# ActiveVisionLab/gaussctrl

Measured on AMD Instinct MI355X. Metric: edited views/sec @512x512 (ControlNet denoise + splat render+bwd), higher is better.
Workload: dtype bf16

## Files before the change

gaussctrl_amd/csrc/dn_gemm.hip:

```cpp
#include "dn_gemm_kernels.h"

namespace {

struct GemmVariant {
    int force_mt;
    int use8;
    int convsplit;
    bool no_wg2, no_persist, full_epilogue, no_lean_ln, tap_outer;
    int forced_pw, slice_mt, epi_abl;
    int undefined;
};
GemmVariant decode_variant(int kv)
{
    const auto bit = [kv](int b) { return (kv & b) != 0; };
    const auto field = [kv](int mask, int shift) { return (kv & mask) >> shift; };
    constexpr int flags = GC_GEMM_VAR_K4_ONLY | GC_GEMM_VAR_FORCE_K8 | GC_GEMM_VAR_NO_CONV_SLICES | GC_GEMM_VAR_NO_SMALL_CONV_SLICES | GC_GEMM_VAR_NO_WG2 |
                          GC_GEMM_VAR_NO_PERSIST | GC_GEMM_VAR_FULL_EPILOGUE | GC_GEMM_VAR_NO_LEAN_LN | GC_GEMM_VAR_TAP_OUTER;
    return {field(GC_GEMM_VAR_MT_MASK, GC_GEMM_VAR_MT_SHIFT), bit(GC_GEMM_VAR_K4_ONLY) ? 0 : bit(GC_GEMM_VAR_FORCE_K8) ? 2 : 1,
            bit(GC_GEMM_VAR_NO_CONV_SLICES) ? 0 : bit(GC_GEMM_VAR_NO_SMALL_CONV_SLICES) ? 1 : 2,
            bit(GC_GEMM_VAR_NO_WG2), bit(GC_GEMM_VAR_NO_PERSIST), bit(GC_GEMM_VAR_FULL_EPILOGUE), bit(GC_GEMM_VAR_NO_LEAN_LN), bit(GC_GEMM_VAR_TAP_OUTER),
            field(GC_GEMM_VAR_PW_MASK, GC_GEMM_VAR_PW_SHIFT), field(GC_GEMM_VAR_SLICE_MT_MASK, GC_GEMM_VAR_SLICE_MT_SHIFT), field(GC_GEMM_VAR_EPI_ABL_MASK, GC_GEMM_VAR_EPI_ABL_SHIFT),
            kv & ~(flags | GC_GEMM_VAR_MT_MASK | GC_GEMM_VAR_PW_MASK | GC_GEMM_VAR_SLICE_MT_MASK | GC_GEMM_VAR_EPI_ABL_MASK)};
}

int choose_splits(int64_t blocks, int nk)
{
    if (blocks >= 128 || nk < 32) return 1;
    int s = (int)((448 + blocks - 1) / blocks);
    if (s > nk / 8) s = nk / 8;
    if (s > 16) s = 16;
    return s < 2 ? 1 : s;
}

int choose_mt(int64_t M, int64_t N, int ntw, bool forced)
{
// ... 200 lines not shown
}

extern "C" int gc_dn_gemm_chan_parts_layout(const gc_gemm_desc *d, int64_t *rows_per_slab, int *nslab, int *col_tile)
{
    GC_REQUIRE(d && rows_per_slab && nslab && col_tile, "null argument");
    *rows_per_slab = 0; *nslab = 0; *col_tile = 0;
    if (d->M <= 0 || d->N <= 0 || d->K <= 0 || d->rows_per_batch <= 0) return GC_OK;
    const GemmVariant v = decode_variant(d->kernel_variant);
    Sel sel;
    select(d, v, &sel, true);
    chan_parts_layout(d, v, sel, rows_per_slab, nslab, col_tile);
    return GC_OK;
}

namespace {
struct Route { Sel sel; int lnk, persist; };
void route(const gc_gemm_desc *d, const GemmVariant &v, Route *r)
{
    Sel &sel = r->sel;
    select(d, v, &sel, d->out_chan_parts != nullptr);
    if (d->out_chan_parts && sel.mt8 == 1) sel.mt8 = 2;
    const bool fuse = d->ln_row_stats || d->out_row_stats || d->out_group_stats;
    r->lnk = (sel.mt8 && sel.splits == 1) ? ln_lean_kind(d, v) : 0;
    r->persist = 0;
    if (sel.mt8 == 4 && sel.ntw == 4 && sel.mode == 0 && sel.splits == 1 && d->K % 64 == 0 && d->K <= 64 * 24 && (!fuse || r->lnk == 2) && !d->out_chan_parts &&
        !d->rowvec && !d->out_t && !d->out_f32 && d->out && d->act != 2 && !v.no_persist) {
        const int64_t tiles = ((d->M + 255) / 256) * ((d->N + 32 * sel.ntw - 1) / (32 * sel.ntw));
        if (tiles > 256) r->persist = 256;
    }
}
}

extern "C" int gc_dn_gemm_selection(const gc_gemm_desc *d, gc_gemm_selection *out)
{
    GC_REQUIRE(d && out, "null argument");
    GC_REQUIRE(d->M > 0 && d->N > 0 && d->K > 0, "empty problem");
    const GemmVariant v = decode_variant(d->kernel_variant);
    if (const int rc = refuse_variant_bits(__func__, v.undefined)) return rc;
    *out = gc_gemm_selection{};
    int64_t rows = 0; int ns = 0, ct = 0;
    if (d->fp8) {
        GC_REQUIRE(d->K % 128 == 0, "fp8: K % 128 == 0");
        SelQ q;
        select_fp8(d, v, &q, false);
        out->kernel = GC_GEMM_SEL_FP8; out->m_tiles = q.mt; out->splits = q.splits; out->ntw = q.ntw;
        if (d->out_chan_parts) {
            chan_parts_layout(d, v, Sel{}, &rows, &ns, &ct);
            out->parts = rows > 0 ? (q.splits > 1 ? 1 : 2) : -1;
        }
        return GC_OK;
    }
    Route r;
    route(d, v, &r);
    out->kernel = !r.sel.mt8 ? GC_GEMM_SEL_K4 : r.sel.splits > 1 ? GC_GEMM_SEL_K8_SLICED : GC_GEMM_SEL_K8;
    out->m_tiles = r.sel.mt8; out->splits = r.sel.splits; out->ntw = r.sel.ntw; out->ln_kind = r.lnk; out->persist = r.persist;
    if (d->out_chan_parts) {
        chan_parts_layout(d, v, r.sel, &rows, &ns, &ct);
        out->parts = rows > 0 ? (r.sel.splits > 1 ? 1 : 2) : -1;
    }
    return GC_OK;
}

extern "C" int gc_dn_gemm(const gc_gemm_desc *d, void *stream)
{
    GC_REQUIRE(d && d->W && d->A, "null descriptor / operand");
    GC_REQUIRE(d->M > 0 && d->N > 0 && d->K > 0, "empty problem");
    GC_REQUIRE(d->K % 8 == 0, "K must be a multiple of 8 (pad channels on the host)");
    GC_REQUIRE(d->N % 4 == 0, "N must be a multiple of 4 (pad output channels on the host)");
    GC_REQUIRE(d->dtype == DT_BF16 || d->dtype == DT_F16, "dtype must be 0 (bf16) or 1 (f16)");
    const GemmVariant v = decode_variant(d->kernel_variant);
// ... 66 lines not shown
        const int ntw = q.ntw, mt = q.mt;
        g.splits = q.splits; g.tiles_per_split = q.tps; g.ws = q.splits > 1 ? (float *)d->workspace : nullptr;
        GC_REQUIRE(!d->out_chan_parts || q.splits > 1 || (d->mode == 1 && !fuse_of(g)), "fp8: channel partials come from k-sliced problems and fast convs");
        const int64_t nbn_q = (d->N + 32 * ntw - 1) / (32 * ntw), nbm_q = (d->M + 64 * mt - 1) / (64 * mt);
        const dim3 gq((unsigned)(nbm_q * nbn_q), (unsigned)q.splits);
        g.pw = pw_of(d, v, nbm_q, nbn_q, nbm_q * nbn_q * q.splits, 32, 64 * mt, 32 * ntw);
        dn_gemm_launch_fp8(g, d->dtype, d->mode == 1 ? 2 : 3, ntw, mt, gq, s);
        if (q.splits > 1) { if (g.chan_parts) dn_gemm_launch_splitk_epilogue_cs(g, d->dtype, s); else dn_gemm_launch_splitk_epilogue(g, d->dtype, s); }
        return gc::check_launch("gc_dn_gemm(fp8)");
    }
    g.splits = sel.splits; g.tiles_per_split = sel.tps; g.ws = (float *)d->workspace;
    const int bn = 32 * sel.ntw;
    const int64_t nbn = (d->N + bn - 1) / bn;
    g.persist = rt.persist;
    const int lnk = rt.lnk;
    if (d->w_set_rows > 0 || d->softmax_keys > 0) {
        GC_REQUIRE(lnk != 0, "weight sets / softmax_keys need a lean LayerNorm-fold problem (K % 64 == 0 linear with ln_row_stats or out_row_stats, no forced variant)");
        GC_REQUIRE(d->w_set_rows == 0 || (d->w_set_rows % (64 * sel.mt8) == 0 && d->M % d->w_set_rows == 0), "w_set_rows must be a multiple of the row tile and divide M");
    }
    if (sel.mt8) {
        const int64_t nbm8 = (d->M + 64 * sel.mt8 - 1) / (64 * sel.mt8);
        const dim3 grid8((unsigned)(nbm8 * nbn), (unsigned)sel.splits);
        g.pw = pw_of(d, v, nbm8, nbn, g.persist ? 8 * 32 : nbm8 * nbn * sel.splits, sel.mt8 == 1 ? 64 : 32, 64 * sel.mt8, bn);
        if (lnk) dn_gemm_launch_ln(g, d->dtype, lnk, lean_of(g, sel.mode) && g.persist == 0, sel.ntw, sel.mt8, grid8, s);
        else if (fuse_of(g)) dn_gemm_launch_fuse(g, d->dtype, sel.mode, sel.ntw, sel.mt8 < 2 ? 2 : sel.mt8, grid8, s);
        else if (g.chan_parts && sel.splits == 1) dn_gemm_launch_cs(g, d->dtype, sel.mode, sel.ntw, sel.mt8, grid8, s);
        else if (lean_of(g, sel.mode) && g.persist == 0 && !v.full_epilogue) dn_gemm_launch_lean(g, d->dtype, sel.mode, sel.ntw, sel.mt8, grid8, s);
        else dn_gemm_launch_plain(g, d->dtype, sel.mode, sel.ntw, sel.mt8, grid8, s);
    } else {
        const int64_t nbm = (d->M + BM - 1) / BM;
        const dim3 grid((unsigned)(nbm * nbn), (unsigned)sel.splits);
        g.pw = pw_of(d, v, nbm, nbn, nbm * nbn * sel.splits, 64, BM, bn);
        if (fuse_of(g)) dn_gemm_launch_fuse(g, d->dtype, sel.mode, sel.ntw, 0, grid, s); else dn_gemm_launch_plain(g, d->dtype, sel.mode, sel.ntw, 0, grid, s);
    }
    if (sel.splits > 1) { if (g.chan_parts) dn_gemm_launch_splitk_epilogue_cs(g, d->dtype, s); else dn_gemm_launch_splitk_epilogue(g, d->dtype, s); }
    return gc::check_launch("gc_dn_gemm");
}
```

gaussctrl_amd/csrc/dn_gemm_kernels.h:

```cpp
#pragma once
#include "dn_common.h"
#include <type_traits>

namespace dng {
struct GemmArgs {
    int64_t M, N, K;
    const void *A; int64_t lda;
    int B, Hi, Wi, Cin, Ho, Wo, stride, ups, pad;
    const void *W;
    const float *bias;
    const float *rowvec; int64_t ld_rowvec; int64_t rows_per_batch;
    const void *residual; int64_t ldr;
    float out_scale;
    int act, geglu;
    void *out; int64_t ldc; int out_f32;
    void *out_t; int64_t ldt; int64_t t_batch_stride; int64_t t_col0;
    int splits; int tiles_per_split;
    int persist;
    float *ws;
    const void *zeros;
    const float *row_stats; int row_stat_slots; const float *colsum; float ln_eps, ln_inv_k;
    float *out_row_stats;
    float *out_group_stats;
    int gn_groups, gn_cpg;
// ... 640 lines not shown
__device__ __forceinline__ void glds16_s(const void *sbase, unsigned voff, unsigned lds_dst)
{
    asm volatile("s_mov_b32 m0, %2\n\ts_nop 0\n\tglobal_load_lds_dwordx4 %0, %1" :: "v"(voff), "s"(sbase), "s"(lds_dst) : "memory");
}

template <class T, int MODE, int NTW, int MT, bool FUSE, bool CS = false, bool LEAN_ = false, int LNV = 0>
__global__ __launch_bounds__(512, MT <= 2 ? 2 : 1) void k_gemm8(const GemmArgs g)
{
    static_assert(!(FUSE && CS), "one statistics epilogue at a time");
    static_assert(LNV == 0 || (!FUSE && !CS && MODE == 3), "lean LayerNorm fold: K % 64 == 0 linears on the non-FUSE epilogues");
    static_assert(LNV != 1 || LEAN_, "row partials come from the lean epilogue");
    static_assert(LNV != 3 || (NTW == 5 && !LEAN_), "softmax-heads epilogue: one 80-column head block per wave column");
    constexpr bool LNIN = LNV >= 2;
    constexpr bool LEAN = LEAN_ || CS;
    constexpr int BM = 64 * MT;
    constexpr bool CONVF = MODE == 2 || MODE == 4, UPS = MODE == 4;
    constexpr int BN = 32 * NTW;
    constexpr int STAGE = BM * 128 + BN * 128;
    constexpr int NS = 3;
    constexpr int AG = BM / 8, WG = BN / 8;
    constexpr int AI = AG / 8, WI = (WG + 7) / 8;
    extern __shared__ __attribute__((aligned(16))) unsigned char smem[];
    const int tid = threadIdx.x, lane = tid & 63;
    const int wid = __builtin_amdgcn_readfirstlane(tid >> 6);
    const int wm = wid >> 1, wn = wid & 1;
    const int nbn = (int)((g.N + BN - 1) / BN);
    int64_t mblk, nblk;
    int slice;
    wg_tile(g, (int)((g.M + BM - 1) / BM), nbn, mblk, nblk, slice);
    const int64_t m_base = mblk * BM, n_base = nblk * BN;
    const int nk_all = (int)((g.K + BK - 1) / BK);
    const int kt0 = slice * g.tiles_per_split;
    const int nk = min(nk_all, kt0 + g.tiles_per_split) - kt0;
    const unsigned lds0 = (unsigned)(size_t)(__attribute__((address_space(3))) unsigned char *)smem;
    float *srow = reinterpret_cast<float *>(smem + NS * STAGE);
    if constexpr (FUSE) {
        if (g.row_stats && g.splits == 1) row_stats_prologue<BM>(g, m_base, srow);
    }
    float *ctab = reinterpret_cast<float *>(smem + NS * STAGE);
    if constexpr (CS) {
        for (int i = tid; i < 4 * BN; i += 512) ctab[i] = 0.f;
    }

    const int lr = lane >> 3, ls = lane & 7;
    int a_off[AI], a_y[AI], a_x[AI], a_ck[AI];
    bool a_ok[AI];
#pragma unroll
    for (int i = 0; i < AI; ++i) {
        const int row = (wid + 8 * i) * 8 + lr;
        a_ck[i] = ls ^ ((row >> 1) & 7);
        const int64_t m = m_base + row;
        a_ok[i] = m < g.M;
        const int mm = a_ok[i] ? (int)m : 0;
        if (MODE == 1 || CONVF) {
            const int hw = g.Ho * g.Wo;
            const int b = mm / hw;
            const int rem = mm - b * hw;
            const int oy = rem / g.Wo;
            a_y[i] = oy * g.stride - g.pad; a_x[i] = (rem - oy * g.Wo) * g.stride - g.pad;
            a_off[i] = b * g.Hi * g.Wi * g.Cin + (CONVF ? a_ck[i] * 8 : 0);
            if (MODE == 2) a_off[i] += (a_y[i] * g.Wi + a_x[i]) * g.Cin;
        } else {
            a_off[i] = mm * (int)g.lda + a_ck[i] * 8;
            if (MODE == 3) a_off[i] = (int)(m < g.M ? m : g.M - 1) * (int)g.lda + a_ck[i] * 8;
            a_y[i] = a_x[i] = 0;
        }
    }
    int w_off[WI], w_ck[WI];
    bool w_ok[WI];
#pragma unroll
    for (int i = 0; i < WI; ++i) {
        const int grp = wid + 8 * i;
        const int row = grp * 8 + lr;
        w_ck[i] = ls ^ ((row >> 1) & 7);
        const int64_t n = n_base + row;
        w_ok[i] = grp < WG && n < g.N;
        w_off[i] = (w_ok[i] ? (int)n : 0) * (int)g.K + w_ck[i] * 8;
        if (MODE == 3) w_off[i] = (int)(n < g.N ? n : g.N - 1) * (int)g.K + w_ck[i] * 8;
    }
    const bool ups = CONVF ? UPS : (g.ups != 0);
    const int Hin = ups ? g.Hi * 2 : g.Hi, Win = ups ? g.Wi * 2 : g.Wi;
    const unsigned char *a_ptr[AI];
    unsigned a_vm[AI];
    if (MODE == 2) {
#pragma unroll
        for (int i = 0; i < AI; ++i) {
            a_ptr[i] = (const unsigned char *)g.A + (int64_t)a_off[i] * 2;
            unsigned vm = 0;
#pragma unroll
            for (int tp = 0; tp < 9; ++tp) {
                const int yi = a_y[i] + tp / 3, xi = a_x[i] + tp % 3;
                if (a_ok[i] && (unsigned)yi < (unsigned)Hin && (unsigned)xi < (unsigned)Win) vm |= 1u << tp;
            }
            a_vm[i] = vm;
        }
    }
    const int64_t wset = (LNV != 0 && g.w_set_rows > 0) ? m_base / g.w_set_rows : 0;
    const unsigned char *Ab = (const unsigned char *)g.A, *Wb = (const unsigned char *)g.W + (LNV != 0 ? wset * g.w_set_stride * 2 : 0);
    const unsigned char *Zp = (const unsigned char *)g.zeros;
    const bool tap_inner = CONVF && g.conv_korder != 0;
    const KOrder kord(tap_inner, BK, g.Cin);
    KCur cur0 = {0, 0};
    if (CONVF && kt0 > 0) cur0 = kord.at(kt0, BK, g.Cin);

    struct TileSrc { int kb, dy_u, dx_u, tap_off, tap; unsigned sbase; KCur next; };
    auto issue_begin = [&](int kt, int stage, const KCur c) __attribute__((always_inline)) -> TileSrc {
        TileSrc t;
        t.kb = (kt0 + kt) * BK; t.dy_u = 0; t.dx_u = 0; t.tap_off = 0; t.tap = 0; t.next = c;
        if (CONVF) {
            const int ci = kord.ci(c);
            t.tap = kord.tap(c);
            t.kb = __builtin_amdgcn_readfirstlane(t.tap * g.Cin + ci);
            t.dy_u = t.tap / 3; t.dx_u = t.tap - t.dy_u * 3;
            t.tap_off = UPS ? ci : (t.dy_u * g.Wi + t.dx_u) * g.Cin + ci;
            t.next = kord.next(c);
        }
        t.sbase = lds0 + stage * STAGE;
        return t;
    };
    auto issue_a = [&](const TileSrc &t, int i) __attribute__((always_inline)) {
        const unsigned dst = t.sbase + (unsigned)((wid + 8 * i) * 1024);
        if (MODE == 3) { glds16_s(Ab + (size_t)t.kb * 2, (unsigned)(a_off[i] * 2), dst); return; }
        if (MODE == 2) {
            const bool okm = (a_vm[i] >> t.tap) & 1u;
            glds16(okm ? a_ptr[i] + (int64_t)t.tap_off * 2 : Zp, dst);
            return;
        }
        bool ok;
        int off;
        if (MODE == 4) {
            int yi = a_y[i] + t.dy_u, xi = a_x[i] + t.dx_u;
            ok = a_ok[i] && (unsigned)yi < (unsigned)Hin && (unsigned)xi < (unsigned)Win;
            off = a_off[i] + t.tap_off;
// ... 5 lines not shown
            const int ci = kc - tap * g.Cin;
            const int dy = tap / 3, dx = tap - dy * 3;
            int yi = a_y[i] + dy, xi = a_x[i] + dx;
            ok = a_ok[i] && k0 < (int)g.K && (unsigned)yi < (unsigned)Hin && (unsigned)xi < (unsigned)Win;
            if (g.ups) { yi >>= 1; xi >>= 1; }
            off = a_off[i] + (yi * g.Wi + xi) * g.Cin + ci;
        } else {
            ok = a_ok[i] && (t.kb + a_ck[i] * 8) < (int)g.K;
            off = a_off[i] + t.kb;
        }
        const unsigned char *src = ok ? Ab + (size_t)(unsigned)(off * 2) : Zp;
        glds16(src, dst);
    };
    auto issue_w = [&](const TileSrc &t, int i, bool has) __attribute__((always_inline)) {
        if (has) {
            const unsigned dst = t.sbase + (unsigned)(BM * 128 + (wid + 8 * i) * 1024);
            if (MODE == 3 || CONVF) { glds16_s(Wb + (size_t)t.kb * 2, (unsigned)(w_off[i] * 2), dst); return; }
            const bool ok = w_ok[i] && (t.kb + w_ck[i] * 8) < (int)g.K;
            const unsigned char *src = ok ? Wb + (size_t)(unsigned)((w_off[i] + t.kb) * 2) : Zp;
            glds16(src, dst);
        }
    };
    auto issue = [&](int kt, int stage, const KCur c) __attribute__((always_inline)) -> KCur {
        const TileSrc t = issue_begin(kt, stage, c);
#pragma unroll
        for (int i = 0; i < AI; ++i) issue_a(t, i);
#pragma unroll
        for (int i = 0; i < WI; ++i) issue_w(t, i, wid + 8 * i < WG);
        return t.next;
    };

// ... 4 lines not shown
        for (int b = 0; b < MT; ++b) acc[a][b] = f32x4{0.f, 0.f, 0.f, 0.f};
    const int fr = lane & 15, fc = lane >> 4;
    const int swz = (fr >> 1) & 7;
    const int fx0 = ((fc ^ swz) << 4), fx1 = (((fc + 4) ^ swz) << 4);
    const int aw0 = BM * 128 + (wn * (16 * NTW) + fr) * 128, aa0 = (wm * (16 * MT) + fr) * 128;
    struct Frag { uint4 w[NTW], a[MT]; };
    auto load_frag = [&](Frag &f, int stage, int ks) __attribute__((always_inline)) {
        const unsigned char *sb = smem + stage * STAGE;
        const int fx = ks ? fx1 : fx0;
#pragma unroll
        for (int t = 0; t < NTW; ++t) f.w[t] = *reinterpret_cast<const uint4 *>(sb + aw0 + fx + t * 2048);
#pragma unroll
        for (int t = 0; t < MT; ++t) f.a[t] = *reinterpret_cast<const uint4 *>(sb + aa0 + fx + t * 2048);
    };
    constexpr int NMM = NTW * MT, NPC = AI + WI;
    auto block = [&](const Frag &f, Frag &fn, int st_next, int ks_next, bool load_next, const TileSrc &t, auto dma_tag, auto w3_tag) __attribute__((always_inline)) {
        constexpr bool DMA = decltype(dma_tag)::value, W3 = decltype(w3_tag)::value;
        static_for<0, NMM>([&](auto m_) __attribute__((always_inline)) {
            constexpr int m = decltype(m_)::value, nt = m / MT, mt = m % MT;
            acc[nt][mt] = T::mfma(f.w[nt], f.a[mt], acc[nt][mt]);
            if constexpr (m == 0) {
                __builtin_amdgcn_sched_barrier(0);
                if (load_next) load_frag(fn, st_next, ks_next);
                __builtin_amdgcn_sched_barrier(0);
            } else if constexpr (DMA && m >= 2) {
                static_for<0, NPC>([&](auto p_) __attribute__((always_inline)) {
                    constexpr int pp = decltype(p_)::value;
                    if constexpr (m == 2 + (pp * (NMM - 3)) / NPC) {
                        __builtin_amdgcn_sched_barrier(0);
                        if constexpr (pp < AI) issue_a(t, pp); else issue_w(t, pp - AI, (pp - AI) < WI - 1 || W3 || WG % 8 == 0);
                        __builtin_amdgcn_sched_barrier(0);
                    }
                });
            }
        });
    };

    const bool w3 = (wid + 8 * (WI - 1)) < WG;
    Frag f0, f1;
    const TileSrc tnone = {0, 0, 0, 0, 0, 0u, {0, 0}};
    auto run = [&](auto w3_tag) __attribute__((always_inline)) {
        constexpr bool W3 = decltype(w3_tag)::value;
        constexpr int GRPW = AI + ((W3 || WG % 8 == 0) ? WI : WI - 1);
        static_assert(2 * GRPW < 64, "vmcnt range");
        auto wait_tiles = [&](auto n_) __attribute__((always_inline)) {
            asm volatile("s_waitcnt vmcnt(%0)" ::"n"(decltype(n_)::value * GRPW) : "memory");
        };
        KCur cur = issue(0, 0, cur0);
        if (nk > 1) cur = issue(1, 1, cur);
        if (nk > 2) cur = issue(2, 2, cur);
// ... 14 lines not shown
            st = st1;
        }
        for (; kt < nk; ++kt) {
            const int st1 = st + 1 == NS ? 0 : st + 1;
            block(f0, f1, st, 1, true, tnone, std::false_type{}, w3_tag);
            const bool more = kt + 1 < nk;
            if (more) {
                if (kt + 2 < nk) wait_tiles(std::integral_constant<int, 1>{}); else wait_tiles(std::integral_constant<int, 0>{});
                asm volatile("s_waitcnt lgkmcnt(0)" ::: "memory");
                __builtin_amdgcn_s_barrier();
            }
            block(f1, f0, st1, 0, more, tnone, std::false_type{}, w3_tag);
            st = st1;
        }
    };
    if (w3) run(std::true_type{}); else run(std::false_type{});

    if constexpr (FUSE) {
        wave_epilogue<T, NTW, MT, 512>(g, acc, m_base, m_base + wm * (16 * MT), n_base + wn * (16 * NTW), lane, smem,
                                       (g.row_stats && g.splits == 1) ? srow : nullptr, slice);
        return;
    }
    const int64_t n_lane = n_base + wn * (16 * NTW) + fc * 4;
    if (g.splits > 1) {
#pragma unroll
        for (int mt = 0; mt < MT; ++mt) {
            const int64_t m = m_base + wm * (16 * MT) + mt * 16 + fr;
            if (m >= g.M) continue;
#pragma unroll
            for (int nt = 0; nt < NTW; ++nt) {
                const int64_t n = n_lane + nt * 16;
// ... 1064 lines not shown
    if (ntw == 5) with_mt(std::integral_constant<int, 5>{}); else with_mt(std::integral_constant<int, 4>{});
}

template <class T, int MODE, int NTW, bool FUSE>
void launch4(const GemmArgs &g, dim3 grid, hipStream_t s)
{
    constexpr size_t lds = 2 * (BM * 128 + 32 * NTW * 128);
    static gc::AttrOnce once;
    gc::ensure_dynamic_lds(once, (const void *)k_gemm<T, MODE, NTW, FUSE>, (int)lds);
    hipLaunchKernelGGL((k_gemm<T, MODE, NTW, FUSE>), grid, dim3(NT), lds, s, g);
}

template <class T, int MODE, int NTW, int MT, bool FUSE, bool CS = false, bool LEAN = false, int LNV = 0>
void launch8(const GemmArgs &g, dim3 grid, hipStream_t s)
{
    constexpr size_t lds = 3 * (64 * MT * 128 + 32 * NTW * 128) + ((FUSE || LNV >= 2) ? 64 * MT * 8 : 0) + (CS ? 32 * NTW * 16 : 0);
    static_assert(lds <= 160 * 1024, "LDS ring");
    static gc::AttrOnce once;
    gc::ensure_dynamic_lds(once, (const void *)k_gemm8<T, MODE, NTW, MT, FUSE, CS, LEAN, LNV>, (int)lds);
    hipLaunchKernelGGL((k_gemm8<T, MODE, NTW, MT, FUSE, CS, LEAN, LNV>), grid, dim3(512), lds, s, g);
}

inline bool ln_lean_producer_of(const GemmArgs &g, int mode, int splits)
{
    return g.out_row_stats && !g.row_stats && !g.out_group_stats && !g.chan_parts && splits == 1 && mode == 0 && g.K % 64 == 0 && !g.geglu &&
           g.act == 0 && !g.out_f32 && !g.out_t && g.out && g.N >= 4 && (!g.rowvec || g.rows_per_batch >= 256);
}
inline bool ln_lean_consumer_of(const GemmArgs &g, int mode, int splits)
{
    return g.row_stats && !g.out_row_stats && !g.out_group_stats && !g.chan_parts && splits == 1 && mode == 0 && g.K % 64 == 0 && g.N >= 4;
}
// ... 11 lines not shown
    if (lnv == 2 && g.persist > 0 && ntw == 4 && mt == 4) { launch8p<T, 4, 4, 2>(g, g.persist, s); return; }
    if (mt == 1 && ntw == 4) { dispatch8ln_m<T, 4, 1>(g, lnv, lean, grid, s); return; }
    with_wave_tile(ntw, mt, [&](auto ntw_, auto mt_) { dispatch8ln_m<T, decltype(ntw_)::value, decltype(mt_)::value>(g, lnv, lean, grid, s); });
}

inline bool lean_of(const GemmArgs &g, int mode)
{
    return !g.geglu && g.act == 0 && !g.out_f32 && !g.out_t && g.out && mode != 1 && (mode != 0 || g.K % 64 == 0) && g.N >= 4 &&
           (!g.rowvec || g.rows_per_batch >= 256);
}
template <class T, int NTW, int MT>
void dispatch8lean_m(const GemmArgs &g, int mode, dim3 grid, hipStream_t s)
{
    if (mode == 0) launch8<T, 3, NTW, MT, false, false, true>(g, grid, s);
    else if (g.ups) launch8<T, 4, NTW, MT, false, false, true>(g, grid, s);
    else launch8<T, 2, NTW, MT, false, false, true>(g, grid, s);
}
template <class T>
void dispatch8lean(const GemmArgs &g, int mode, int ntw, int mt, dim3 grid, hipStream_t s)
{
    if (mt == 1 && ntw == 4 && mode == 0) { launch8<T, 3, 4, 1, false, false, true>(g, grid, s); return; }
    with_wave_tile(ntw, mt, [&](auto ntw_, auto mt_) { dispatch8lean_m<T, decltype(ntw_)::value, decltype(mt_)::value>(g, mode, grid, s); });
}

template <class T, int NTW, int MT>
void dispatch8cs_m(const GemmArgs &g, int mode, dim3 grid, hipStream_t s)
{
    if (mode == 0) launch8<T, 3, NTW, MT, false, true>(g, grid, s);
    else if (mode == 1) launch8<T, 1, NTW, MT, false, true>(g, grid, s);
    else launch8<T, 2, NTW, MT, false, true>(g, grid, s);
}
template <class T>
void dispatch8cs(const GemmArgs &g, int mode, int ntw, int mt, dim3 grid, hipStream_t s)
{
    with_wave_tile(ntw, mt, [&](auto ntw_, auto mt_) { dispatch8cs_m<T, decltype(ntw_)::value, decltype(mt_)::value>(g, mode, grid, s); });
}

template <class T, int NTW, int MT, bool FUSE>
void dispatch8m(const GemmArgs &g, int mode, dim3 grid, hipStream_t s)
{
    if constexpr (FUSE) {
        if (mode == 0) launch8<T, 3, NTW, MT, true>(g, grid, s);
        else if (mode == 1) launch8<T, 1, NTW, MT, true>(g, grid, s);
        else launch8<T, 2, NTW, MT, true>(g, grid, s);
    } else {
        if (mode == 0) { if (g.K % 64 == 0) launch8<T, 3, NTW, MT, false>(g, grid, s); else launch8<T, 0, NTW, MT, false>(g, grid, s); }
        else if (mode == 1) launch8<T, 1, NTW, MT, false>(g, grid, s);
        else if (g.ups) launch8<T, 4, NTW, MT, false>(g, grid, s); else launch8<T, 2, NTW, MT, false>(g, grid, s);
    }
}
template <class T, bool FUSE>
void dispatch8(const GemmArgs &g, int mode, int ntw, int mt, dim3 grid, hipStream_t s)
{
    if constexpr (!FUSE) {
        if (mt == 1 && ntw == 4 && mode == 0 && g.K % 64 == 0) { launch8<T, 3, 4, 1, false>(g, grid, s); return; }
        if (g.persist > 0 && ntw == 4 && mt == 4 && mode == 0) { launch8p<T, 4, 4>(g, g.persist, s); return; }
    }
    with_wave_tile(ntw, mt, [&](auto ntw_, auto mt_) { dispatch8m<T, decltype(ntw_)::value, decltype(mt_)::value, FUSE>(g, mode, grid, s); });
}

template <class T, bool FUSE>
void dispatch4(const GemmArgs &g, int mode, int ntw, dim3 grid, hipStream_t s)
{
// ... 19 lines not shown
```

gaussctrl_amd/sd/ops.py:

```python
from __future__ import annotations

import ctypes as C
import dataclasses
import os
import sys
import types

import torch

from .. import _lib as L


class GemmDesc(C.Structure):
    _fields_ = [("dtype", C.c_int), ("mode", C.c_int), ("M", C.c_int64), ("N", C.c_int64), ("K", C.c_int64),
                ("A", C.c_void_p), ("lda", C.c_int64),
                ("B", C.c_int), ("Hi", C.c_int), ("Wi", C.c_int), ("Cin", C.c_int), ("Ho", C.c_int), ("Wo", C.c_int),
                ("stride", C.c_int), ("upsample", C.c_int), ("pad_lo", C.c_int),
                ("W", C.c_void_p), ("bias", C.c_void_p), ("rowvec", C.c_void_p), ("ld_rowvec", C.c_int64),
                ("rows_per_batch", C.c_int64), ("residual", C.c_void_p), ("ldr", C.c_int64), ("out_scale", C.c_float),
                ("act", C.c_int), ("geglu", C.c_int), ("out", C.c_void_p), ("ldc", C.c_int64), ("out_f32", C.c_int),
                ("out_t", C.c_void_p), ("ldt", C.c_int64), ("t_batch_stride", C.c_int64), ("t_col0", C.c_int64),
                ("workspace", C.c_void_p), ("workspace_bytes", C.c_size_t), ("zeros", C.c_void_p),
                ("ln_row_stats", C.c_void_p), ("ln_row_stat_slots", C.c_int), ("ln_colsum", C.c_void_p), ("ln_eps", C.c_float),
                ("out_row_stats", C.c_void_p), ("out_group_stats", C.c_void_p), ("gn_groups", C.c_int),
# ... 4 lines not shown

class AttnDesc(C.Structure):
    _fields_ = [("dtype", C.c_int), ("batch", C.c_int), ("heads", C.c_int), ("head_dim", C.c_int), ("Lq", C.c_int),
                ("Lk", C.c_int), ("frames_per_half", C.c_int), ("nsets", C.c_int), ("set_kind", C.c_int * 5),
                ("set_weight", C.c_float * 5), ("scale", C.c_float),
                ("Q", C.c_void_p), ("ldq", C.c_int64), ("q_batch_stride", C.c_int64),
                ("K", C.c_void_p), ("ldk", C.c_int64), ("k_batch_stride", C.c_int64),
                ("Vt", C.c_void_p), ("ldvt", C.c_int64), ("vt_batch_stride", C.c_int64),
                ("O", C.c_void_p), ("ldo", C.c_int64), ("o_batch_stride", C.c_int64),
                ("Kref", C.c_void_p), ("kref_batch_stride", C.c_int64), ("Vtref", C.c_void_p),
                ("vtref_batch_stride", C.c_int64), ("ref_frames_per_half", C.c_int), ("q_prescaled", C.c_int),
                ("kernel_variant", C.c_int), ("workspace", C.c_void_p), ("workspace_bytes", C.c_size_t)]


class GemmSelection(C.Structure):
    _fields_ = [(n, C.c_int) for n in ("kernel", "m_tiles", "splits", "ntw", "parts", "ln_kind", "persist")]


GEMM_KERNELS = {1: "k4", 2: "k8", 3: "k8_sliced", 4: "fp8"}
ATTN_KERNELS = {1: "attn5", 2: "attn4", 3: "attn3", 4: "wide+combine", 5: "attn+combine", 6: "attn"}

GC_GEMM_VAR_MT_MASK, GC_GEMM_VAR_MT_SHIFT = 0x7, 0
GC_GEMM_VAR_K4_ONLY, GC_GEMM_VAR_FORCE_K8, GC_GEMM_VAR_NO_CONV_SLICES, GC_GEMM_VAR_NO_SMALL_CONV_SLICES = 0x10, 0x20, 0x40, 0x80
GC_GEMM_VAR_NO_WG2, GC_GEMM_VAR_NO_PERSIST, GC_GEMM_VAR_FULL_EPILOGUE, GC_GEMM_VAR_NO_LEAN_LN, GC_GEMM_VAR_TAP_OUTER = 0x100, 0x200, 0x400, 0x800, 0x1000
GC_GEMM_VAR_PW_MASK, GC_GEMM_VAR_PW_SHIFT = 0xff0000, 16
GC_GEMM_VAR_SLICE_MT_MASK, GC_GEMM_VAR_SLICE_MT_SHIFT = 0x7000000, 24
GC_GEMM_VAR_EPI_ABL_MASK, GC_GEMM_VAR_EPI_ABL_SHIFT = 0x70000000, 28
GC_ATTN_VAR_ONLINE_ONLY, GC_ATTN_VAR_D40_K3, GC_ATTN_VAR_K4_8WAVE, GC_ATTN_VAR_K4_Q64, GC_ATTN_VAR_K4 = 1, 2, 4, 8, 16
GC_ATTN_VAR_RING4, GC_ATTN_VAR_RING8, GC_ATTN_VAR_D160_Q64 = 32, 64, 128
GC_ATTN_VAR_ABL_MASK, GC_ATTN_VAR_ABL_SHIFT = 0xff00, 8
GC_ATTN_VAR_CSHIFT_MASK, GC_ATTN_VAR_CSHIFT_SHIFT = 0x1f0000, 16


def gemm_selection(d):
    sel = GemmSelection()
    L.check(L.lib().gc_dn_gemm_selection(C.byref(d), C.byref(sel)), "gc_dn_gemm_selection")
    r = {n: getattr(sel, n) for n, _ in GemmSelection._fields_}
    r["kernel"] = GEMM_KERNELS[sel.kernel]
    return r


# ... 610 lines not shown
```

include/gaussctrl_hip.h:

```cpp
#ifndef GAUSSCTRL_HIP_H
#define GAUSSCTRL_HIP_H

#include <stddef.h>
#include <stdint.h>

#ifdef __cplusplus
extern "C" {
#endif

#define GC_OK 0
#define GC_EINVAL (-1)
#define GC_ELAUNCH (-2)
#define GC_ENOSPC (-3)

const char *gc_last_error_string(void);
int gc_abi_version(void);


int gc_project_gaussians_fwd(int64_t N, const float *means3d, const float *scales, float glob_scale,
                             const float *quats, const float *viewmat, const float *projmat,
                             float fx, float fy, float cx, float cy, int img_h, int img_w,
                             int tiles_x, int tiles_y, float clip_thresh,
                             float *cov3d, float *xys, float *depths, int32_t *radii, float *conics,
                             int32_t *num_tiles_hit, void *stream);
// ... 187 lines not shown


enum { GC_GEMM_VAR_MT_MASK = 0x7, GC_GEMM_VAR_MT_SHIFT = 0,
       GC_GEMM_VAR_K4_ONLY = 0x10,
       GC_GEMM_VAR_FORCE_K8 = 0x20,
       GC_GEMM_VAR_NO_CONV_SLICES = 0x40,
       GC_GEMM_VAR_NO_SMALL_CONV_SLICES = 0x80,
       GC_GEMM_VAR_NO_WG2 = 0x100,
       GC_GEMM_VAR_NO_PERSIST = 0x200,
       GC_GEMM_VAR_FULL_EPILOGUE = 0x400,
       GC_GEMM_VAR_NO_LEAN_LN = 0x800,
       GC_GEMM_VAR_TAP_OUTER = 0x1000,
       GC_GEMM_VAR_PW_MASK = 0xff0000, GC_GEMM_VAR_PW_SHIFT = 16,
       GC_GEMM_VAR_SLICE_MT_MASK = 0x7000000, GC_GEMM_VAR_SLICE_MT_SHIFT = 24,
       GC_GEMM_VAR_EPI_ABL_MASK = 0x70000000, GC_GEMM_VAR_EPI_ABL_SHIFT = 28 };
typedef struct gc_gemm_desc {
    int dtype;
    int mode;
    int64_t M, N, K;
    const void *A;
    int64_t lda;
    int B, Hi, Wi, Cin, Ho, Wo, stride, upsample;
    int pad_lo;
    const void *W;
    const float *bias;
    const float *rowvec;
    int64_t ld_rowvec;
    int64_t rows_per_batch;
    const void *residual;
    int64_t ldr;
// ... 30 lines not shown
size_t gc_dn_gemm_workspace_bytes(const gc_gemm_desc *desc);
int gc_dn_gemm_row_stat_slots(const gc_gemm_desc *desc);
int gc_dn_gemm_chan_parts_layout(const gc_gemm_desc *desc, int64_t *rows_per_slab, int *nslab, int *col_tile);
enum { GC_GEMM_SEL_K4 = 1,
       GC_GEMM_SEL_K8 = 2,
       GC_GEMM_SEL_K8_SLICED = 3,
       GC_GEMM_SEL_FP8 = 4 };
typedef struct gc_gemm_selection {
    int kernel;
    int m_tiles;
    int splits;
    int ntw;
    int parts;
    int ln_kind;
    int persist;
} gc_gemm_selection;
int gc_dn_gemm_selection(const gc_gemm_desc *desc, gc_gemm_selection *out);
int gc_dn_gemm(const gc_gemm_desc *desc, void *stream);

enum { GC_ATTN_VAR_ONLINE_ONLY = 1,
       GC_ATTN_VAR_D40_K3 = 2,
       GC_ATTN_VAR_K4_8WAVE = 4,
       GC_ATTN_VAR_K4_Q64 = 8,
       GC_ATTN_VAR_K4 = 16,
       GC_ATTN_VAR_RING4 = 32, GC_ATTN_VAR_RING8 = 64,
       GC_ATTN_VAR_D160_Q64 = 128,
       GC_ATTN_VAR_ABL_MASK = 0xff00, GC_ATTN_VAR_ABL_SHIFT = 8,
       GC_ATTN_VAR_CSHIFT_MASK = 0x1f0000, GC_ATTN_VAR_CSHIFT_SHIFT = 16 };
typedef struct gc_attn_desc {
    int dtype;
// ... 111 lines not shown
```

Measured before the change: 11.57.

## Share 3x3 conv A-tile rows across horizontal taps via shifted LDS reads

Adds a row-share conv mode for 3x3 stride-1 same-padded convolutions whose row tile is a multiple of the image width. Each A slab is loaded once per kernel row into LDS, and the three horizontal taps read it at shifted row offsets, with edge lanes zeroed. Only the weight tiles rotate through the three-stage ring. The aim is to cut A-operand global loads and LDS traffic by about three times for these convs. In exchange it adds a new kernel instantiation with a custom barrier and waitcnt schedule, and it is restricted to non-fused epilogues and to slicing where the tiles per split are a multiple of 3.

```diff
diff --git a/gaussctrl_amd/csrc/dn_gemm.hip b/gaussctrl_amd/csrc/dn_gemm.hip
--- a/gaussctrl_amd/csrc/dn_gemm.hip
+++ b/gaussctrl_amd/csrc/dn_gemm.hip
@@ -7,6 +7,7 @@
     int use8;
     int convsplit;
     bool no_wg2, no_persist, full_epilogue, no_lean_ln, tap_outer;
+    bool no_row_share;
     int forced_pw, slice_mt, epi_abl;
     int undefined;
 };
@@ -19,6 +20,7 @@
     return {field(GC_GEMM_VAR_MT_MASK, GC_GEMM_VAR_MT_SHIFT), bit(GC_GEMM_VAR_K4_ONLY) ? 0 : bit(GC_GEMM_VAR_FORCE_K8) ? 2 : 1,
             bit(GC_GEMM_VAR_NO_CONV_SLICES) ? 0 : bit(GC_GEMM_VAR_NO_SMALL_CONV_SLICES) ? 1 : 2,
             bit(GC_GEMM_VAR_NO_WG2), bit(GC_GEMM_VAR_NO_PERSIST), bit(GC_GEMM_VAR_FULL_EPILOGUE), bit(GC_GEMM_VAR_NO_LEAN_LN), bit(GC_GEMM_VAR_TAP_OUTER),
+            field(GC_GEMM_VAR_SLICE_MT_MASK, GC_GEMM_VAR_SLICE_MT_SHIFT) == GC_GEMM_SLICE_MT_NO_ROW_SHARE,
             field(GC_GEMM_VAR_PW_MASK, GC_GEMM_VAR_PW_SHIFT), field(GC_GEMM_VAR_SLICE_MT_MASK, GC_GEMM_VAR_SLICE_MT_SHIFT), field(GC_GEMM_VAR_EPI_ABL_MASK, GC_GEMM_VAR_EPI_ABL_SHIFT),
             kv & ~(flags | GC_GEMM_VAR_MT_MASK | GC_GEMM_VAR_PW_MASK | GC_GEMM_VAR_SLICE_MT_MASK | GC_GEMM_VAR_EPI_ABL_MASK)};
 }
@@ -249,7 +251,14 @@
 }
 
 namespace {
-struct Route { Sel sel; int lnk, persist; };
+struct Route { Sel sel; int lnk, persist; bool row_share; };
+bool row_share_of(const gc_gemm_desc *d, const GemmVariant &v, const Sel &sel, bool fuse)
+{
+    if (sel.mode != 2 || sel.mt8 < 2 || fuse || v.tap_outer || v.no_row_share) return false;
+    if (d->upsample || d->stride != 1 || d->pad_lo != 1 || d->Hi != d->Ho || d->Wi != d->Wo || d->Wo < 1) return false;
+    if ((64 * sel.mt8) % d->Wo != 0) return false;
+    return sel.splits == 1 || sel.tps % 3 == 0;
+}
 void route(const gc_gemm_desc *d, const GemmVariant &v, Route *r)
 {
     Sel &sel = r->sel;
@@ -263,6 +272,7 @@
         const int64_t tiles = ((d->M + 255) / 256) * ((d->N + 32 * sel.ntw - 1) / (32 * sel.ntw));
         if (tiles > 256) r->persist = 256;
     }
+    r->row_share = row_share_of(d, v, sel, fuse);
 }
 }
 
@@ -288,7 +298,7 @@
     Route r;
     route(d, v, &r);
     out->kernel = !r.sel.mt8 ? GC_GEMM_SEL_K4 : r.sel.splits > 1 ? GC_GEMM_SEL_K8_SLICED : GC_GEMM_SEL_K8;
-    out->m_tiles = r.sel.mt8; out->splits = r.sel.splits; out->ntw = r.sel.ntw; out->ln_kind = r.lnk; out->persist = r.persist;
+    out->m_tiles = r.sel.mt8; out->splits = r.sel.splits; out->ntw = r.sel.ntw; out->ln_kind = r.lnk; out->persist = r.persist; out->conv_row_share = r.row_share;
     if (d->out_chan_parts) {
         chan_parts_layout(d, v, r.sel, &rows, &ns, &ct);
         out->parts = rows > 0 ? (r.sel.splits > 1 ? 1 : 2) : -1;
@@ -385,6 +395,7 @@
     const int64_t nbn = (d->N + bn - 1) / bn;
     g.persist = rt.persist;
     const int lnk = rt.lnk;
+    const int kmode = rt.row_share ? 5 : sel.mode;
     if (d->w_set_rows > 0 || d->softmax_keys > 0) {
         GC_REQUIRE(lnk != 0, "weight sets / softmax_keys need a lean LayerNorm-fold problem (K % 64 == 0 linear with ln_row_stats or out_row_stats, no forced variant)");
         GC_REQUIRE(d->w_set_rows == 0 || (d->w_set_rows % (64 * sel.mt8) == 0 && d->M % d->w_set_rows == 0), "w_set_rows must be a multiple of the row tile and divide M");
@@ -395,9 +406,9 @@
         g.pw = pw_of(d, v, nbm8, nbn, g.persist ? 8 * 32 : nbm8 * nbn * sel.splits, sel.mt8 == 1 ? 64 : 32, 64 * sel.mt8, bn);
         if (lnk) dn_gemm_launch_ln(g, d->dtype, lnk, lean_of(g, sel.mode) && g.persist == 0, sel.ntw, sel.mt8, grid8, s);
         else if (fuse_of(g)) dn_gemm_launch_fuse(g, d->dtype, sel.mode, sel.ntw, sel.mt8 < 2 ? 2 : sel.mt8, grid8, s);
-        else if (g.chan_parts && sel.splits == 1) dn_gemm_launch_cs(g, d->dtype, sel.mode, sel.ntw, sel.mt8, grid8, s);
-        else if (lean_of(g, sel.mode) && g.persist == 0 && !v.full_epilogue) dn_gemm_launch_lean(g, d->dtype, sel.mode, sel.ntw, sel.mt8, grid8, s);
-        else dn_gemm_launch_plain(g, d->dtype, sel.mode, sel.ntw, sel.mt8, grid8, s);
+        else if (g.chan_parts && sel.splits == 1) dn_gemm_launch_cs(g, d->dtype, kmode, sel.ntw, sel.mt8, grid8, s);
+        else if (lean_of(g, sel.mode) && g.persist == 0 && !v.full_epilogue) dn_gemm_launch_lean(g, d->dtype, kmode, sel.ntw, sel.mt8, grid8, s);
+        else dn_gemm_launch_plain(g, d->dtype, kmode, sel.ntw, sel.mt8, grid8, s);
     } else {
         const int64_t nbm = (d->M + BM - 1) / BM;
         const dim3 grid((unsigned)(nbm * nbn), (unsigned)sel.splits);
diff --git a/gaussctrl_amd/csrc/dn_gemm_kernels.h b/gaussctrl_amd/csrc/dn_gemm_kernels.h
--- a/gaussctrl_amd/csrc/dn_gemm_kernels.h
+++ b/gaussctrl_amd/csrc/dn_gemm_kernels.h
@@ -678,10 +678,14 @@
     constexpr bool LNIN = LNV >= 2;
     constexpr bool LEAN = LEAN_ || CS;
     constexpr int BM = 64 * MT;
-    constexpr bool CONVF = MODE == 2 || MODE == 4, UPS = MODE == 4;
+    constexpr bool RS = MODE == 5, M2 = MODE == 2 || RS;
+    constexpr bool CONVF = M2 || MODE == 4, UPS = MODE == 4;
+    static_assert(!RS || !FUSE, "row share: the plain, lean and channel-partial epilogues");
     constexpr int BN = 32 * NTW;
     constexpr int STAGE = BM * 128 + BN * 128;
     constexpr int NS = 3;
+    constexpr int WST = BN * 128, ASLOT = BM * 128, A0 = 128, W0 = RS ? A0 + 2 * ASLOT + 128 : 0;
+    constexpr int RING = RS ? W0 + NS * WST : NS * STAGE;
     constexpr int AG = BM / 8, WG = BN / 8;
     constexpr int AI = AG / 8, WI = (WG + 7) / 8;
     extern __shared__ __attribute__((aligned(16))) unsigned char smem[];
@@ -697,11 +701,11 @@
     const int kt0 = slice * g.tiles_per_split;
     const int nk = min(nk_all, kt0 + g.tiles_per_split) - kt0;
     const unsigned lds0 = (unsigned)(size_t)(__attribute__((address_space(3))) unsigned char *)smem;
-    float *srow = reinterpret_cast<float *>(smem + NS * STAGE);
+    float *srow = reinterpret_cast<float *>(smem + RING);
     if constexpr (FUSE) {
         if (g.row_stats && g.splits == 1) row_stats_prologue<BM>(g, m_base, srow);
     }
-    float *ctab = reinterpret_cast<float *>(smem + NS * STAGE);
+    float *ctab = reinterpret_cast<float *>(smem + RING);
     if constexpr (CS) {
         for (int i = tid; i < 4 * BN; i += 512) ctab[i] = 0.f;
     }
@@ -723,7 +727,7 @@
             const int oy = rem / g.Wo;
             a_y[i] = oy * g.stride - g.pad; a_x[i] = (rem - oy * g.Wo) * g.stride - g.pad;
             a_off[i] = b * g.Hi * g.Wi * g.Cin + (CONVF ? a_ck[i] * 8 : 0);
-            if (MODE == 2) a_off[i] += (a_y[i] * g.Wi + a_x[i]) * g.Cin;
+            if (M2) a_off[i] += (a_y[i] * g.Wi + a_x[i]) * g.Cin;
         } else {
             a_off[i] = mm * (int)g.lda + a_ck[i] * 8;
             if (MODE == 3) a_off[i] = (int)(m < g.M ? m : g.M - 1) * (int)g.lda + a_ck[i] * 8;
@@ -746,14 +750,14 @@
     const int Hin = ups ? g.Hi * 2 : g.Hi, Win = ups ? g.Wi * 2 : g.Wi;
     const unsigned char *a_ptr[AI];
     unsigned a_vm[AI];
-    if (MODE == 2) {
+    if (M2) {
 #pragma unroll
         for (int i = 0; i < AI; ++i) {
             a_ptr[i] = (const unsigned char *)g.A + (int64_t)a_off[i] * 2;
             unsigned vm = 0;
 #pragma unroll
-            for (int tp = 0; tp < 9; ++tp) {
-                const int yi = a_y[i] + tp / 3, xi = a_x[i] + tp % 3;
+            for (int tp = 0; tp < (RS ? 3 : 9); ++tp) {
+                const int yi = a_y[i] + (RS ? tp : tp / 3), xi = a_x[i] + (RS ? 1 : tp % 3);
                 if (a_ok[i] && (unsigned)yi < (unsigned)Hin && (unsigned)xi < (unsigned)Win) vm |= 1u << tp;
             }
             a_vm[i] = vm;
@@ -779,8 +783,12 @@
             t.tap_off = UPS ? ci : (t.dy_u * g.Wi + t.dx_u) * g.Cin + ci;
             t.next = kord.next(c);
         }
-        t.sbase = lds0 + stage * STAGE;
+        t.sbase = lds0 + (RS ? W0 + stage * WST : stage * STAGE);
         return t;
+    };
+    auto issue_a_rs = [&](const TileSrc &t, int i, int slot) __attribute__((always_inline)) {
+        const bool okm = (a_vm[i] >> t.dy_u) & 1u;
+        glds16(okm ? a_ptr[i] + (int64_t)(t.tap_off + g.Cin) * 2 : Zp, lds0 + (unsigned)(A0 + slot + (wid + 8 * i) * 1024));
     };
     auto issue_a = [&](const TileSrc &t, int i) __attribute__((always_inline)) {
         const unsigned dst = t.sbase + (unsigned)((wid + 8 * i) * 1024);
@@ -816,7 +824,7 @@
     };
     auto issue_w = [&](const TileSrc &t, int i, bool has) __attribute__((always_inline)) {
         if (has) {
-            const unsigned dst = t.sbase + (unsigned)(BM * 128 + (wid + 8 * i) * 1024);
+            const unsigned dst = t.sbase + (unsigned)((RS ? 0 : BM * 128) + (wid + 8 * i) * 1024);
             if (MODE == 3 || CONVF) { glds16_s(Wb + (size_t)t.kb * 2, (unsigned)(w_off[i] * 2), dst); return; }
             const bool ok = w_ok[i] && (t.kb + w_ck[i] * 8) < (int)g.K;
             const unsigned char *src = ok ? Wb + (size_t)(unsigned)((w_off[i] + t.kb) * 2) : Zp;
@@ -851,26 +859,37 @@
         for (int t = 0; t < MT; ++t) f.a[t] = *reinterpret_cast<const uint4 *>(sb + aa0 + fx + t * 2048);
     };
     constexpr int NMM = NTW * MT, NPC = AI + WI;
-    auto block = [&](const Frag &f, Frag &fn, int st_next, int ks_next, bool load_next, const TileSrc &t, auto dma_tag, auto w3_tag) __attribute__((always_inline)) {
-        constexpr bool DMA = decltype(dma_tag)::value, W3 = decltype(w3_tag)::value;
+    auto block_of = [&](Frag &f, auto npc_tag, auto &&edge, auto &&next, auto &&piece) __attribute__((always_inline)) {
+        constexpr int NP = decltype(npc_tag)::value;
         static_for<0, NMM>([&](auto m_) __attribute__((always_inline)) {
             constexpr int m = decltype(m_)::value, nt = m / MT, mt = m % MT;
+            if constexpr (nt == 0) edge(f, std::integral_constant<int, mt>{});
             acc[nt][mt] = T::mfma(f.w[nt], f.a[mt], acc[nt][mt]);
             if constexpr (m == 0) {
                 __builtin_amdgcn_sched_barrier(0);
-                if (load_next) load_frag(fn, st_next, ks_next);
+                next();
                 __builtin_amdgcn_sched_barrier(0);
-            } else if constexpr (DMA && m >= 2) {
-                static_for<0, NPC>([&](auto p_) __attribute__((always_inline)) {
+            } else if constexpr (NP > 0 && m >= 2) {
+                static_for<0, NP>([&](auto p_) __attribute__((always_inline)) {
                     constexpr int pp = decltype(p_)::value;
-                    if constexpr (m == 2 + (pp * (NMM - 3)) / NPC) {
+                    if constexpr (m == 2 + (pp * (NMM - 3)) / NP) {
                         __builtin_amdgcn_sched_barrier(0);
-                        if constexpr (pp < AI) issue_a(t, pp); else issue_w(t, pp - AI, (pp - AI) < WI - 1 || W3 || WG % 8 == 0);
+                        piece(p_);
                         __builtin_amdgcn_sched_barrier(0);
                     }
                 });
             }
         });
+    };
+    auto no_edge = [](Frag &, auto) __attribute__((always_inline)) {};
+    auto block = [&](Frag &f, Frag &fn, int st_next, int ks_next, bool load_next, const TileSrc &t, auto dma_tag, auto w3_tag) __attribute__((always_inline)) {
+        constexpr bool DMA = decltype(dma_tag)::value, W3 = decltype(w3_tag)::value;
+        block_of(f, std::integral_constant<int, DMA ? NPC : 0>{}, no_edge,
+                 [&]() __attribute__((always_inline)) { if (load_next) load_frag(fn, st_next, ks_next); },
+                 [&](auto p_) __attribute__((always_inline)) {
+                     constexpr int pp = decltype(p_)::value;
+                     if constexpr (pp < AI) issue_a(t, pp); else issue_w(t, pp - AI, (pp - AI) < WI - 1 || W3 || WG % 8 == 0);
+                 });
     };
 
     const bool w3 = (wid + 8 * (WI - 1)) < WG;
@@ -915,7 +934,97 @@
             st = st1;
         }
     };
-    if (w3) run(std::true_type{}); else run(std::false_type{});
+    int ab[3];
+    bool edge_l[MT], edge_r[MT];
+    if constexpr (RS) {
+#pragma unroll
+        for (int s = 0; s < 3; ++s) ab[s] = A0 + (wm * (16 * MT) + fr + s - 1) * 128 + ((fc ^ (((fr + s - 1) >> 1) & 7)) << 4);
+#pragma unroll
+        for (int t = 0; t < MT; ++t) {
+            const int x = (wm * (16 * MT) + t * 16 + fr) % g.Wo;
+            edge_l[t] = x == 0; edge_r[t] = x == g.Wo - 1;
+        }
+    }
+    auto load_frag_rs = [&](Frag &f, int ws, int slot, int s, int ks) __attribute__((always_inline)) {
+        const unsigned char *sw = smem + W0 + ws * WST + (wn * (16 * NTW) + fr) * 128 + (ks ? fx1 : fx0);
+        const unsigned char *sa = smem + slot + (ab[s] ^ (ks ? 64 : 0));
+#pragma unroll
+        for (int t = 0; t < NTW; ++t) f.w[t] = *reinterpret_cast<const uint4 *>(sw + t * 2048);
+#pragma unroll
+        for (int t = 0; t < MT; ++t) f.a[t] = *reinterpret_cast<const uint4 *>(sa + t * 2048);
+    };
+    auto run_rs = [&](auto w3_tag) __attribute__((always_inline)) {
+        constexpr bool W3 = decltype(w3_tag)::value;
+        constexpr int WIw = (W3 || WG % 8 == 0) ? WI : WI - 1;
+        static_assert(AI + 2 * WIw < 64, "vmcnt range");
+        auto wait_dma = [&](auto n_) __attribute__((always_inline)) { asm volatile("s_waitcnt vmcnt(%0)" ::"n"(decltype(n_)::value) : "memory"); };
+        auto sync = [&]() __attribute__((always_inline)) {
+            asm volatile("s_waitcnt lgkmcnt(0)" ::: "memory");
+            __builtin_amdgcn_s_barrier();
+        };
+        auto zero_l = [&](Frag &f, auto mt_) __attribute__((always_inline)) { if (edge_l[decltype(mt_)::value]) f.a[decltype(mt_)::value] = make_uint4(0u, 0u, 0u, 0u); };
+        auto zero_r = [&](Frag &f, auto mt_) __attribute__((always_inline)) { if (edge_r[decltype(mt_)::value]) f.a[decltype(mt_)::value] = make_uint4(0u, 0u, 0u, 0u); };
+        auto no_piece = [](auto) __attribute__((always_inline)) {};
+        constexpr std::integral_constant<int, 0> none{};
+        auto triple = [&](int slot, KCur cur, auto more_tag) __attribute__((always_inline)) -> KCur {
+            constexpr bool MORE = decltype(more_tag)::value;
+            const int nslot = slot ^ ASLOT;
+            TileSrc t = tnone;
+            auto w_piece = [&](auto p_) __attribute__((always_inline)) {
+                constexpr int pp = decltype(p_)::value;
+                issue_w(t, pp, pp < WI - 1 || W3 || WG % 8 == 0);
+            };
+            auto aw_piece = [&](auto p_) __attribute__((always_inline)) {
+                constexpr int pp = decltype(p_)::value;
+                if constexpr (pp < AI) issue_a_rs(t, pp, nslot); else issue_w(t, pp - AI, (pp - AI) < WI - 1 || W3 || WG % 8 == 0);
+            };
+            block_of(f0, none, zero_l, [&]() __attribute__((always_inline)) { load_frag_rs(f1, 0, slot, 0, 1); }, no_piece);
+            wait_dma(std::integral_constant<int, WIw>{});
+            sync();
+            if constexpr (MORE) { t = issue_begin(0, 0, cur); cur = t.next; }
+            block_of(f1, std::integral_constant<int, MORE ? NPC : 0>{}, zero_l, [&]() __attribute__((always_inline)) { load_frag_rs(f0, 1, slot, 1, 0); }, aw_piece);
+            block_of(f0, none, no_edge, [&]() __attribute__((always_inline)) { load_frag_rs(f1, 1, slot, 1, 1); }, no_piece);
+            wait_dma(std::integral_constant<int, MORE ? AI + WIw : 0>{});
+            sync();
+            if constexpr (MORE) { t = issue_begin(0, 1, cur); cur = t.next; }
+            block_of(f1, std::integral_constant<int, MORE ? WI : 0>{}, no_edge, [&]() __attribute__((always_inline)) { load_frag_rs(f0, 2, slot, 2, 0); }, w_piece);
+            block_of(f0, none, zero_r, [&]() __attribute__((always_inline)) { load_frag_rs(f1, 2, slot, 2, 1); }, no_piece);
+            if constexpr (MORE) {
+                wait_dma(std::integral_constant<int, WIw>{});
+                sync();
+                t = issue_begin(0, 2, cur); cur = t.next;
+            }
+            block_of(f1, std::integral_constant<int, MORE ? WI : 0>{}, zero_r, [&]() __attribute__((always_inline)) { if constexpr (MORE) load_frag_rs(f0, 0, nslot, 0, 0); }, w_piece);
+            return cur;
+        };
+        KCur cur = cur0;
+        {
+            TileSrc t = issue_begin(0, 0, cur);
+            cur = t.next;
+#pragma unroll
+            for (int i = 0; i < AI; ++i) issue_a_rs(t, i, 0);
+#pragma unroll
+            for (int i = 0; i < WI; ++i) issue_w(t, i, wid + 8 * i < WG);
+#pragma unroll
+            for (int st = 1; st < 3; ++st) {
+                t = issue_begin(0, st, cur);
+                cur = t.next;
+#pragma unroll
+                for (int i = 0; i < WI; ++i) issue_w(t, i, wid + 8 * i < WG);
+            }
+        }
+        wait_dma(std::integral_constant<int, 2 * WIw>{});
+        __builtin_amdgcn_s_barrier();
+        load_frag_rs(f0, 0, 0, 0, 0);
+        int slot = 0;
+        for (int p = 3; p < nk; p += 3) {
+            cur = triple(slot, cur, std::true_type{});
+            slot ^= ASLOT;
+        }
+        triple(slot, cur, std::false_type{});
+    };
+    if constexpr (RS) { if (w3) run_rs(std::true_type{}); else run_rs(std::false_type{}); }
+    else { if (w3) run(std::true_type{}); else run(std::false_type{}); }
 
     if constexpr (FUSE) {
         wave_epilogue<T, NTW, MT, 512>(g, acc, m_base, m_base + wm * (16 * MT), n_base + wn * (16 * NTW), lane, smem,
@@ -2010,7 +2119,8 @@
 template <class T, int MODE, int NTW, int MT, bool FUSE, bool CS = false, bool LEAN = false, int LNV = 0>
 void launch8(const GemmArgs &g, dim3 grid, hipStream_t s)
 {
-    constexpr size_t lds = 3 * (64 * MT * 128 + 32 * NTW * 128) + ((FUSE || LNV >= 2) ? 64 * MT * 8 : 0) + (CS ? 32 * NTW * 16 : 0);
+    constexpr size_t ring = MODE == 5 ? 256 + 2 * (64 * MT * 128) + 3 * (32 * NTW * 128) : 3 * (64 * MT * 128 + 32 * NTW * 128);
+    constexpr size_t lds = ring + ((FUSE || LNV >= 2) ? 64 * MT * 8 : 0) + (CS ? 32 * NTW * 16 : 0);
     static_assert(lds <= 160 * 1024, "LDS ring");
     static gc::AttrOnce once;
     gc::ensure_dynamic_lds(once, (const void *)k_gemm8<T, MODE, NTW, MT, FUSE, CS, LEAN, LNV>, (int)lds);
@@ -2052,6 +2162,7 @@
 {
     if (mode == 0) launch8<T, 3, NTW, MT, false, false, true>(g, grid, s);
     else if (g.ups) launch8<T, 4, NTW, MT, false, false, true>(g, grid, s);
+    else if (mode == 5) launch8<T, 5, NTW, MT, false, false, true>(g, grid, s);
     else launch8<T, 2, NTW, MT, false, false, true>(g, grid, s);
 }
 template <class T>
@@ -2066,6 +2177,7 @@
 {
     if (mode == 0) launch8<T, 3, NTW, MT, false, true>(g, grid, s);
     else if (mode == 1) launch8<T, 1, NTW, MT, false, true>(g, grid, s);
+    else if (mode == 5) launch8<T, 5, NTW, MT, false, true>(g, grid, s);
     else launch8<T, 2, NTW, MT, false, true>(g, grid, s);
 }
 template <class T>
@@ -2084,7 +2196,9 @@
     } else {
         if (mode == 0) { if (g.K % 64 == 0) launch8<T, 3, NTW, MT, false>(g, grid, s); else launch8<T, 0, NTW, MT, false>(g, grid, s); }
         else if (mode == 1) launch8<T, 1, NTW, MT, false>(g, grid, s);
-        else if (g.ups) launch8<T, 4, NTW, MT, false>(g, grid, s); else launch8<T, 2, NTW, MT, false>(g, grid, s);
+        else if (g.ups) launch8<T, 4, NTW, MT, false>(g, grid, s);
+        else if (mode == 5) launch8<T, 5, NTW, MT, false>(g, grid, s);
+        else launch8<T, 2, NTW, MT, false>(g, grid, s);
     }
 }
 template <class T, bool FUSE>
diff --git a/gaussctrl_amd/sd/ops.py b/gaussctrl_amd/sd/ops.py
--- a/gaussctrl_amd/sd/ops.py
+++ b/gaussctrl_amd/sd/ops.py
@@ -42,7 +42,7 @@
 
 
 class GemmSelection(C.Structure):
-    _fields_ = [(n, C.c_int) for n in ("kernel", "m_tiles", "splits", "ntw", "parts", "ln_kind", "persist")]
+    _fields_ = [(n, C.c_int) for n in ("kernel", "m_tiles", "splits", "ntw", "parts", "ln_kind", "persist", "conv_row_share")]
 
 
 GEMM_KERNELS = {1: "k4", 2: "k8", 3: "k8_sliced", 4: "fp8"}
@@ -53,6 +53,7 @@
 GC_GEMM_VAR_NO_WG2, GC_GEMM_VAR_NO_PERSIST, GC_GEMM_VAR_FULL_EPILOGUE, GC_GEMM_VAR_NO_LEAN_LN, GC_GEMM_VAR_TAP_OUTER = 0x100, 0x200, 0x400, 0x800, 0x1000
 GC_GEMM_VAR_PW_MASK, GC_GEMM_VAR_PW_SHIFT = 0xff0000, 16
 GC_GEMM_VAR_SLICE_MT_MASK, GC_GEMM_VAR_SLICE_MT_SHIFT = 0x7000000, 24
+GC_GEMM_SLICE_MT_NO_ROW_SHARE = 7
 GC_GEMM_VAR_EPI_ABL_MASK, GC_GEMM_VAR_EPI_ABL_SHIFT = 0x70000000, 28
 GC_ATTN_VAR_ONLINE_ONLY, GC_ATTN_VAR_D40_K3, GC_ATTN_VAR_K4_8WAVE, GC_ATTN_VAR_K4_Q64, GC_ATTN_VAR_K4 = 1, 2, 4, 8, 16
 GC_ATTN_VAR_RING4, GC_ATTN_VAR_RING8, GC_ATTN_VAR_D160_Q64 = 32, 64, 128
diff --git a/include/gaussctrl_hip.h b/include/gaussctrl_hip.h
--- a/include/gaussctrl_hip.h
+++ b/include/gaussctrl_hip.h
@@ -225,6 +225,7 @@
        GC_GEMM_VAR_PW_MASK = 0xff0000, GC_GEMM_VAR_PW_SHIFT = 16,
        GC_GEMM_VAR_SLICE_MT_MASK = 0x7000000, GC_GEMM_VAR_SLICE_MT_SHIFT = 24,
        GC_GEMM_VAR_EPI_ABL_MASK = 0x70000000, GC_GEMM_VAR_EPI_ABL_SHIFT = 28 };
+enum { GC_GEMM_SLICE_MT_NO_ROW_SHARE = 7 };
 typedef struct gc_gemm_desc {
     int dtype;
     int mode;
@@ -285,6 +286,7 @@
     int parts;
     int ln_kind;
     int persist;
+    int conv_row_share;
 } gc_gemm_selection;
 int gc_dn_gemm_selection(const gc_gemm_desc *desc, gc_gemm_selection *out);
 int gc_dn_gemm(const gc_gemm_desc *desc, void *stream);
```

Result: no change. 11.50 (-0.6%).
